# stevengiacalone/triceratops

Hardware: AMD Instinct MI355X
Metric: light-curve-point x sample evals/sec (higher is better)
Workload: dtype f64

## Files before the change

include/trx_debug.h:

```cpp
#ifndef TRX_DEBUG_H
#define TRX_DEBUG_H

#include "trx.h"

#ifdef __cplusplus
extern "C" {
#endif

int trx_set_rows_per_wave(int rows);
int trx_set_cell_packing_below(int n_time);
int trx_debug_batch_plan(long rows, int rows_per_wave, int taper, long* positions, int* rows_min);

int trx_set_supersample_tiers(int on);
int trx_set_stencil(int on);
int trx_set_skip_excluded(int on);
int trx_set_debug_node_counts(int on);
int trx_set_kepler_stepping(int on);

int trx_set_bounded_evaluation(int mode);
int trx_set_debug_bounded_lnl(int on);
int trx_set_debug_poison(int on);
int trx_set_debug_bug(int on);
int trx_set_probe_rows(int rows);
int trx_set_star_chain(int on);
int trx_set_row_order(int on);
int trx_debug_row_order(long* n_rows, long* segment_capacity, int* counts, int* lists, double* row_blocks);
int trx_set_whole_trips(int on);
int trx_debug_whole_trips(long* whole, long* walked, int reset);
int trx_debug_chain_counts(long* chains, long* calls_in_chains, long* posterior_calls_in_chains, int reset);

int trx_debug_select_from_halfchi2(const double* halfchi2, const double* lnprior, const double* cols,
                                   const double* cols_pad, long n, long N, long n_total, int ncol, int twin, int K,
                                   int moments, double lnsigma, double* out_record, double* out_post_x,
                                   double* out_table, void* stream);

int trx_debug_capture_buffers(long* live, long* idle);

#ifdef __cplusplus
}
#endif
#endif
```

triceratops_amd/_lib.py:

```python
import ctypes
import os
import threading

import numpy as np
import torch

_HERE = os.path.dirname(os.path.abspath(__file__))
LIB_PATH = os.environ.get("TRX_LIB") or os.path.join(_HERE, "libtrx.so")
TESTING_LIB_PATH = os.environ.get("TRX_TESTING_LIB") or os.path.join(_HERE, "libtrx_testing.so")

MODEL_TP, MODEL_EB, MODEL_EB_TWIN, MODEL_RAW = 0, 1, 2, 3
FLAG_COMPANION_IS_HOST, FLAG_SCALAR_K, FLAG_FP32_MODEL, FLAG_EVALUATE_EXCLUDED = 1, 2, 4, 8
FLAG_ALL_SUBEXPOSURES, FLAG_NO_STENCIL, FLAG_COUNT_EVALUATIONS, FLAG_FULL_EVALUATION = 16, 32, 64, 128
FLAG_WEIGHT_MOMENTS = 256
N_PARAM = {MODEL_TP: 10, MODEL_EB: 11, MODEL_EB_TWIN: 11, MODEL_RAW: 9}
ERR_NTOTAL = 4

ABI_SYMBOLS = (
    "trx_lnl_batch", "trx_lnl_batch_weighted", "trx_flux_grid", "trx_chi2_grid", "trx_chi2_grid_weighted",
    "trx_chi2_grid_offset", "trx_chi2_grid_baseline", "trx_workspace_bytes",
    "trx_log_mean_exp", "trx_lnz_scenario", "trx_lnz_from_halfchi2", "trx_lnz_moments_from_halfchi2",
    "trx_posterior_from_halfchi2", "trx_grid_quantiles",
    "trx_lnl_batch_host", "trx_flux_grid_host",
    "trx_log_mean_exp_host", "trx_skipped_rows", "trx_pruned_rows",
    "trx_draw_scenario", "trx_draw_args_size", "trx_scenario_evidence", "trx_scenario_enqueue", "trx_star_enqueue",
    "trx_scenario_args_size", "trx_release_scratch", "trx_version", "trx_last_error", "trx_device_count",
)
WARP_SYMBOLS = ("trxw_hist_from_halfchi2",)
NOISE_SYMBOLS = ("trxn_chi2_grid_ou",)
MIX_SYMBOLS = ("trxm_chi2_grid_ou_mix",)
SHIFT_SYMBOLS = ("trxt_softmin_rows",)
DEBUG_SYMBOLS = (
    "trx_set_rows_per_wave", "trx_set_cell_packing_below", "trx_debug_batch_plan", "trx_set_supersample_tiers",
    "trx_set_stencil", "trx_set_skip_excluded", "trx_set_debug_node_counts", "trx_set_kepler_stepping",
    "trx_set_bounded_evaluation", "trx_set_debug_bounded_lnl", "trx_set_debug_poison", "trx_set_debug_bug",
    "trx_set_probe_rows", "trx_set_star_chain", "trx_debug_capture_buffers", "trx_debug_chain_counts",
    "trx_set_row_order", "trx_debug_row_order", "trx_set_whole_trips", "trx_debug_whole_trips",
    "trx_debug_select_from_halfchi2",
)


class TrxError(RuntimeError):
    pass


EXTRA_FLAGS = 0
CELL_PACKING_BELOW = 320
STATS = {"rows": 0, "cells": 0, "launches": 0, "native_calls": 0}
_stats_lock = threading.Lock()


def count_launch(rows, n_time):
    with _stats_lock:
        STATS["rows"] += rows
        STATS["cells"] += rows * n_time
        STATS["launches"] += 1
TRACE = None
TRACE_SAMPLE_ROWS = 128


def reset_stats():
    for k in STATS:
        STATS[k] = 0


def set_precision(mode):
    global EXTRA_FLAGS
    if mode not in ("fp64", "fp32"):
        raise ValueError("precision must be 'fp64' or 'fp32'")
    EXTRA_FLAGS = (EXTRA_FLAGS & ~FLAG_FP32_MODEL) | (FLAG_FP32_MODEL if mode == "fp32" else 0)


def set_full_evaluation(on):
    global EXTRA_FLAGS
    EXTRA_FLAGS = (EXTRA_FLAGS | FLAG_FULL_EVALUATION) if on else (EXTRA_FLAGS & ~FLAG_FULL_EVALUATION)


_vp = ctypes.c_void_p
_lib = None
_production = None
_testing = None


def lib():
    global _lib, _production
    if _lib is not None:
        return _lib
    if os.environ.get("TRX_TESTING") == "1":
        return use_testing_library(True)
    if _production is None:
# ... 40 lines not shown
    L.trx_chi2_grid_weighted.restype = c_int
    L.trx_chi2_grid_weighted.argtypes = [_vp, _vp, _vp, c_int, c_long, _vp, c_double, c_int, _vp, _vp]
    L.trx_chi2_grid_offset.restype = c_int
    L.trx_chi2_grid_offset.argtypes = [_vp, _vp, _vp, c_int, c_long, _vp, c_double, c_int, _vp, c_double, c_double, _vp,
                                       _vp]
    L.trx_chi2_grid_baseline.restype = c_int
    L.trx_chi2_grid_baseline.argtypes = [_vp, _vp, _vp, c_int, c_long, _vp, c_double, c_int, _vp, _vp, c_int, _vp, _vp,
                                         _vp]
    L.trx_workspace_bytes.restype = c_size_t
    L.trx_workspace_bytes.argtypes = []
    L.trx_log_mean_exp.restype = c_int
    L.trx_log_mean_exp.argtypes = [_vp, c_long, c_long, _vp, _vp, c_size_t, _vp]
    L.trx_lnz_scenario.restype = c_int
    L.trx_lnz_scenario.argtypes = [c_int, c_int, _vp, _vp, c_int, c_double, _vp, c_long, c_double,
                                   c_int, _vp, c_long, c_double, _vp, _vp, _vp, c_size_t, _vp]
    L.trx_lnz_from_halfchi2.restype = c_int
    L.trx_lnz_from_halfchi2.argtypes = [_vp, _vp, c_long, c_long, c_double, _vp, _vp, c_size_t, _vp]
    L.trx_lnz_moments_from_halfchi2.restype = c_int
    L.trx_lnz_moments_from_halfchi2.argtypes = [_vp, _vp, c_long, c_long, c_double, _vp, _vp, c_size_t, _vp]
    L.trx_posterior_from_halfchi2.restype = c_int
    L.trx_posterior_from_halfchi2.argtypes = [_vp, _vp, c_long, c_double, c_int, ctypes.c_ulonglong, _vp, _vp, _vp,
                                              c_size_t, _vp]
    L.trxw_hist_from_halfchi2.restype = c_int
    L.trxw_hist_from_halfchi2.argtypes = [_vp, _vp, _vp, _vp, c_long, c_double, _vp, _vp, c_size_t, _vp]
    L.trxn_chi2_grid_ou.restype = c_int
    L.trxn_chi2_grid_ou.argtypes = [_vp, _vp, c_int, c_long, _vp, c_double, c_int, _vp, _vp, _vp, _vp, _vp]
    L.trxm_chi2_grid_ou_mix.restype = c_int
    L.trxm_chi2_grid_ou_mix.argtypes = [_vp, _vp, c_int, c_long, _vp, c_double, c_int, _vp, _vp, _vp, _vp, c_int, _vp, _vp,
                                        _vp]
    L.trxt_softmin_rows.restype = c_int
    L.trxt_softmin_rows.argtypes = [_vp, c_long, c_long, c_int, _vp, c_int, _vp, _vp]
    L.trx_grid_quantiles.restype = c_int
    L.trx_grid_quantiles.argtypes = [_vp, c_long, c_int, _vp, _vp, c_long, _vp, c_int, _vp, _vp]
    L.trx_lnl_batch_host.restype = c_int
    L.trx_lnl_batch_host.argtypes = [c_int, c_int, _vp, _vp, c_int, c_double, _vp, c_long,
                                     c_double, c_int, _vp]
    L.trx_flux_grid_host.restype = c_int
    L.trx_flux_grid_host.argtypes = [c_int, c_int, _vp, c_int, _vp, c_long, c_double, c_int, _vp, _vp]
    L.trx_log_mean_exp_host.restype = c_int
    L.trx_log_mean_exp_host.argtypes = [_vp, c_long, c_long, _vp]
    L.trx_skipped_rows.restype = c_int
    L.trx_skipped_rows.argtypes = [ctypes.POINTER(ctypes.c_ulonglong), c_int]
    L.trx_pruned_rows.restype = c_int
    L.trx_pruned_rows.argtypes = [ctypes.POINTER(ctypes.c_ulonglong), c_int]
    L.trx_version.restype = ctypes.c_char_p
    L.trx_last_error.restype = ctypes.c_char_p
    L.trx_device_count.restype = c_int
    L.trx_testing = bool(testing)
    if testing:
        for name in ("trx_set_rows_per_wave", "trx_set_kepler_stepping", "trx_set_skip_excluded",
                     "trx_set_bounded_evaluation", "trx_set_debug_bounded_lnl", "trx_set_debug_poison",
                     "trx_set_debug_bug", "trx_set_star_chain", "trx_set_probe_rows", "trx_set_stencil",
                     "trx_set_supersample_tiers", "trx_set_debug_node_counts", "trx_set_cell_packing_below",
                     "trx_set_row_order", "trx_set_whole_trips"):
            fn = getattr(L, name)
            fn.restype = c_int
            fn.argtypes = [c_int]
        L.trx_debug_capture_buffers.restype = c_int
        L.trx_debug_capture_buffers.argtypes = [ctypes.POINTER(c_long), ctypes.POINTER(c_long)]
        L.trx_debug_row_order.restype = c_int
        L.trx_debug_row_order.argtypes = [ctypes.POINTER(c_long), ctypes.POINTER(c_long), _vp, _vp, _vp]
        L.trx_debug_whole_trips.restype = c_int
        L.trx_debug_whole_trips.argtypes = [ctypes.POINTER(c_long), ctypes.POINTER(c_long), c_int]
        L.trx_debug_select_from_halfchi2.restype = c_int
        L.trx_debug_select_from_halfchi2.argtypes = [_vp, _vp, _vp, _vp, c_long, c_long, c_long, c_int, c_int, c_int, c_int,
                                                     c_double, _vp, _vp, _vp, _vp]
    return L


def check(rc):
    if rc:
        msg = lib().trx_last_error().decode()
        if rc == ERR_NTOTAL:
            raise ValueError(msg)
        raise TrxError("libtrx error %d: %s" % (rc, msg))


def version():
    return lib().trx_version().decode()


_gpu_seen = False


def require_gpu():
    global _gpu_seen
    if _gpu_seen:
        return
    if not torch.cuda.is_available() or lib().trx_device_count() < 1:
        raise TrxError("triceratops_amd needs an AMD GPU (gfx950); none is visible and there is no "
                       "CPU fallback")
    _gpu_seen = True
    from . import hw_queues
    if hw_queues()["in_effect"] is False:
        import warnings
        warnings.warn("triceratops_amd was imported after the HIP runtime had been initialised: GPU_MAX_HW_QUEUES=16 "
                      "did not take effect (the runtime keeps its default of 4 hardware queues; calc_probs on more "
                      "than two streams runs ~10 % slower).  Import triceratops_amd before the first GPU call or "
                      "export GPU_MAX_HW_QUEUES=16.", RuntimeWarning, stacklevel=3)


def compute_device():
    require_gpu()
    return torch.device("cuda", torch.cuda.current_device())


_upload_streams = {}
# ... 455 lines not shown
```

triceratops_amd/csrc/trx_cells.hpp:

```cpp
#pragma once
#include <hip/hip_runtime.h>
#include <math.h>

#include <cstddef>
#include <cstdint>

#include "../../include/trx.h"
#include "trx_device.hpp"
#include "trx_internal.hpp"

namespace {

using namespace trx;

constexpr int MODE_LNL = 0;
constexpr int MODE_GRID = 1;

struct RowsArgs {
    int model, flags;
    const double* time;
    const double* flux;
    int n_time;
    double sigma;
    const double* params;
    long n;
    double exptime;
    int S;
    double* out;
    double* out_sec;
    int B;
    long nbatch;
    int use_tiers, debug_nodes;
    int debug_bug;
    int need_sec;
    int mark_unwritten;
    int use_stencil;
    int skip_excl;
    int* memo;
    int tl_off;
    int wave_off, wave_doubles;
    int probe_rows;
    int wave_floor;
    int wave_floor3;
    double* rowc;
    int* scan_list;
    unsigned long long* scan_count;
    const long* n_dev;
    const int* src_idx;
    long src_stride;
    int twin_cols;
    int dense;
    int forced_B;
    int prune;
    int pstride;
    int pstride3;
    double prune_c0;
    const double* prune_lp;
    int part;
    int split;
    int* surv_list;
    unsigned long long* surv_count;
    int* probe_list;
    unsigned long long* probe_count;
    TierHead tiers;
    const double* tier_xw;
    double s2, rs2, dS, rS;
    const double* inv_var;
    double sec_limit;
    int accumulate;
    int whole_trips;
    int* order;
};

#ifndef TRX_CHAIN_MAX_BRANCHES
#define TRX_CHAIN_MAX_BRANCHES 24
#endif
struct BranchArgs {
    int model, flags, twin_cols, need_sec;
    const double* flux;
    double sigma, s2, rs2, prune_c0;
    const double* params;
    double* out;
    const long* n_dev;
    const int* src_idx;
    const double* prune_lp;
    double* scratch;
    unsigned long long* scan_count;
};
constexpr int kChainMaxBranches = TRX_CHAIN_MAX_BRANCHES;
struct BranchTab {
    BranchArgs b[kChainMaxBranches];
};
static_assert(sizeof(RowsArgs) + sizeof(BranchTab) + 16 <= 4096, "kernel argument buffer");

__device__ __forceinline__ double uniform(double v)
{
    const unsigned long long b = __double_as_longlong(v);
    const unsigned lo = __builtin_amdgcn_readfirstlane((unsigned)b);
    const unsigned hi = __builtin_amdgcn_readfirstlane((unsigned)(b >> 32));
    return __longlong_as_double(((unsigned long long)hi << 32) | lo);
}

__device__ __forceinline__ long uniform_long(long v)
{
    const unsigned lo = __builtin_amdgcn_readfirstlane((unsigned)(unsigned long long)v);
    const unsigned hi = __builtin_amdgcn_readfirstlane((unsigned)((unsigned long long)v >> 32));
    return (long)(((unsigned long long)hi << 32) | lo);
}

__device__ __forceinline__ bool mask_bit(unsigned long long m, int i)
{
    const unsigned w = (i & 32) ? (unsigned)(m >> 32) : (unsigned)m;
    return ((w >> (i & 31)) & 1u) != 0u;
}

__device__ __forceinline__ long row_pos(const RowsArgs& a, long row)
{
    if (a.dense) return a.twin_cols ? a.src_stride - 1 - row : row;
    return a.src_idx ? (long)a.src_idx[row] : row;
}

__device__ __forceinline__ int lanes_below(unsigned long long m)
{
    return __builtin_amdgcn_mbcnt_hi((unsigned)(m >> 32), __builtin_amdgcn_mbcnt_lo((unsigned)m, 0u));
}

#ifdef TRX_PHASE_TIMERS
__device__ unsigned long long g_phase_cycles[8];
#define TRX_TICK(var) const unsigned long long var = __builtin_readcyclecounter()
#define TRX_TOCK(slot, from) tm[slot] += __builtin_readcyclecounter() - (from)
#else
#define TRX_TICK(var)
#define TRX_TOCK(slot, from)
#endif

#ifdef TRX_TAIL_TIMERS
constexpr int kTailWaves = 1 << 17;
__device__ unsigned long long g_tail[4] = {~0ull, 0ull, 0ull, 0ull};
__device__ unsigned long long g_tail_finish[kTailWaves];
#endif

constexpr int kStatShards = 256, kStatPad = 16;
__device__ unsigned long long g_row_stats[2][kStatShards][kStatPad];
__device__ __forceinline__ void add_row_stat(int which, unsigned count)
{
    if (count) atomicAdd(&g_row_stats[which][(blockIdx.x + 41u * blockIdx.y) & (kStatShards - 1)][0], (unsigned long long)count);
}

#ifdef TRX_TESTING
__device__ unsigned long long g_trip_stats[2][kStatShards][kStatPad];
__device__ __forceinline__ void add_trip_stat(int which, unsigned count)
{
    if (count) atomicAdd(&g_trip_stats[which][(blockIdx.x + 41u * blockIdx.y) & (kStatShards - 1)][0], (unsigned long long)count);
}
__device__ __forceinline__ bool whole_trips_on(const RowsArgs& a) { return a.whole_trips != 0; }
#define TRX_TRIP_STAT(var) ++var
#else
__device__ __forceinline__ bool whole_trips_on(const RowsArgs&) { return true; }
#define TRX_TRIP_STAT(var)
#endif

__device__ __forceinline__ double k_rule(double k, bool scalar_rule)
{
    if (scalar_rule) { if (fabs(k - 1.0) < 1e-6) k *= 0.999; }
    else             { if ((k - 1.0) < 1e-6) k *= 0.999; }
    return k;
}

#ifndef TRX_BATCH_WAVES
#define TRX_BATCH_WAVES 4
#endif

constexpr int kBatchWaves = TRX_BATCH_WAVES;
__host__ __device__ constexpr int cells_waves(bool long_rows) { return long_rows ? 1 : kBatchWaves; }
#ifndef TRX_TIER_LDS
#define TRX_TIER_LDS(PRUNE, LONG) true
#endif
#ifndef TRX_ATAN_TAB
#define TRX_ATAN_TAB(PRUNE, LONG) (((PRUNE) && !(LONG)) ? 2 : 1)
#endif
#ifndef TRX_LONG_ROWS_IN_LDS
#define TRX_LONG_ROWS_IN_LDS 0
#endif
#ifndef TRX_CARRY_CELLS
#define TRX_CARRY_CELLS 1
#endif
#ifndef TRX_CELLS_WAVES_PER_EU
#define TRX_CELLS_WAVES_PER_EU 4
#endif
#ifndef TRX_LAZY_TIERS
#define TRX_LAZY_TIERS 1
#endif
#ifndef TRX_CELLS_PAIRS
#define TRX_CELLS_PAIRS 640
#endif
#ifndef TRX_CELLS_WINDOW
#define TRX_CELLS_WINDOW 2048
#endif
constexpr int kCellsMaxRows = 22;
#ifndef TRX_CELLS_WINDOW_BATCH
#define TRX_CELLS_WINDOW_BATCH 768
#endif
#ifndef TRX_BATCH_WAVES_PER_EU
#define TRX_BATCH_WAVES_PER_EU 5
#endif
constexpr int kCellsWindowLong = TRX_CELLS_WINDOW, kCellsWindowBatch = TRX_CELLS_WINDOW_BATCH;
static_assert(kCellsWindowLong % 64 == 0 && kCellsWindowLong <= 64 * 64, "window_trips: a lane per trip, windows that begin on a trip");
__host__ __device__ constexpr int cells_window(bool long_rows) { return long_rows ? kCellsWindowLong : kCellsWindowBatch; }
constexpr int kCellsPairs = TRX_CELLS_PAIRS;

__host__ __device__ inline int batch_rows(long n, int n_time, int forced, int floor = 3200)
{
    int B = (640 + n_time / 2) / (n_time > 0 ? n_time : 1);
    B = B < 1 ? 1 : (B > kCellsMaxRows ? kCellsMaxRows : B);
    if (forced > 0) return forced > kCellsMaxRows ? kCellsMaxRows : forced;
    if (n >= 0)
        while (B > 1 && n / B < floor) B = (B + 1) / 2;
    return B;
}

#ifndef TRX_TAPER_SLOTS
#define TRX_TAPER_SLOTS 320
#endif
struct BatchPlan {
    long R;
    long ra, rb;
    long pa, pb, P;
    int B, B2, B3;
};
__host__ __device__ inline BatchPlan batch_plan(long rows, int B, bool taper = true)
{
    BatchPlan p;
    p.B = B;
    p.B2 = (B + 1) / 2;
    p.B3 = B / 4 > 0 ? B / 4 : 1;
    const long nb = (rows + B - 1) / B;
    p.R = ((nb + 7) / 8) * B;
    long rb = 0, rc = 0;
#ifndef TRX_NO_TAPER
    if (B > 1 && taper) {
        constexpr long kSlotsPerXcd = TRX_TAPER_SLOTS;
        rc = kSlotsPerXcd * p.B3;
        if (rc > (3 * p.R) / 20) rc = (3 * p.R) / 20;
        rb = kSlotsPerXcd * p.B2;
        if (rb > (3 * p.R) / 10) rb = (3 * p.R) / 10;
        rc -= rc % B;
        rb -= rb % B;
// ... 878 lines not shown
                const int cell = c0 + lane;
                const bool valid = cell < win1;
                if (ST && !((trips >> ((c0 - win0) >> 6)) & 1ull)) {
                    if (MODE == MODE_GRID && valid) a.out[(size_t)base * n_time + cell] = a.debug_nodes ? 0.0 : hmout[0];
                    continue;
                }
                if (kWholeTrips && ((trips >> (32 + ((c0 - win0) >> 6))) & 1ull)) {
                    if (MODE == MODE_GRID && a.debug_nodes && valid) a.out[(size_t)base * n_time + cell] = 0.0;
                    if (valid) winlist[nw + lanes_below(~0ull)] = (unsigned short)(cell - win0);
                    nw += (win1 - c0 < 64) ? win1 - c0 : 64;
                    TRX_TRIP_STAT(n_whole);
                    continue;
                }
                TRX_TRIP_STAT(n_walked);
                int rr = 0, j = valid ? cell : 0;
                if (!LONG) {
                    rr = valid ? (int)(((float)cell + 0.5f) * inv_nt) : (nb - 1);
                    rr = rr < nb ? rr : nb - 1;
                    j = valid ? (cell - rr * n_time) : 0;
                }
                bool inw = false;
                TRX_CENSUS_ADD(kCenWindowTrip, 1);
                if (PRUNE && !LONG && !__any(valid && !mask_bit(skipmask, rr))) continue;
                if (valid) {
                    const RowC& c = (LONG && !TRX_LONG_ROWS_IN_LDS) ? cu : rows[rr];
                    const double phase = c.nmot * (tl[j] - c.t0);
                    const double dMc = reduce_2pi(phase);
                    const double slack = 1e-15 * fabs(phase);
                    const RowC& cw = rows[rr];
                    inw = in_window(cw.wlo - slack, cw.whi + slack, dMc) && !mask_bit(skipmask, rr);
                    if (MODE == MODE_GRID && (!inw || a.debug_nodes))
                        a.out[(size_t)base * n_time + cell] = a.debug_nodes ? 0.0 : hmout[rr];
                    if (LONG && MODE == MODE_LNL && !inw && phase_no == 0) {
                        const double d = fl[j] - 1.0;
                        lacc = fma(d * d, WT ? wl[j] : rs2, lacc);
                    }
                    if (PRUNE) {
                        if (!LONG && inw && phase_no == 0) {
                            const double d = fl[j] - 1.0;
                            __hip_atomic_fetch_add(&hrem[rr], (d * d) * rs2, __ATOMIC_RELAXED, __HIP_MEMORY_SCOPE_WORKGROUP);
                        }
                        if (nphase == 2) {
                            const bool probe = (j % pstride) == (pstride >> 1);
                            inw = inw && (probe == (phase_no == 0));
                        }
                    }
                }
                const unsigned long long mw = __ballot(inw);
                if (inw) winlist[nw + lanes_below(mw)] = (unsigned short)(cell - win0);
                nw += __popcll(mw);
            }
            wave_sync();
            TRX_TOCK(1, t_p1);
            int nheavy = 0;
            for (int sweep = 0; sweep < 2; ++sweep) {
            const int count = sweep ? nheavy : nw;
            const bool halo = ST && sweep == 0 && st_radius > 0.0;
            int carry_j = 0;
            unsigned long long carry_ok = 0;
            int ncarry = 0;
            for (int w0 = 0, step = 64; w0 < count || (kCarry && ncarry > 0); w0 += step) {
                TRX_TICK(t_plan);
                TRX_CENSUS_ADD(sweep ? kCenChunk1 : kCenChunk0, 1);
                bool owned = true;
                const bool carried = kCarry && lane < ncarry;
                if (kCarry) step = 64 - ncarry;
                const int csrc = (lane + 64 - ncarry) & 63;
                const unsigned cmeta = carried ? cs.meta[csrc] : 0u;
                bool valid = carried ? (cmeta & 0x20000u) != 0 : (w0 + lane - ncarry) < count;
                int rel = (int)*(carried ? &cs.rel[csrc] : &winlist[valid ? (w0 + lane - ncarry) : (count - 1)]);
                bool last_chunk = false;
                if (ST && halo) {
                    last_chunk = w0 + 64 >= count;
                    step = last_chunk ? 64 : 64 - kStM;
                    owned = lane < step;
                    if (w0 > 0 && lane < kStM) ss.fc[lane] = ss.fc[kStM + (64 - 2 * kStM) + lane];
                    wave_sync();
                }
                const int cell = win0 + rel;
                int rr = 0, j = cell;
                if (!LONG) {
                    rr = (int)(((float)cell + 0.5f) * inv_nt);
                    rr = rr < nb ? rr : nb - 1;
                    j = cell - rr * n_time;
                }
                const double t = tl[j];
                double fobs = 0.0;
                if (LONG && MODE == MODE_LNL) fobs = fl[j];
                double wobs = rs2;
                if (LONG && WT) wobs = wl[j];
                CellPlan pl;
                if (carried) {
                    pl.n = (int)(cmeta >> 18); pl.tier = (int)((cmeta >> 8) & 0xffu) - 1;
                    pl.sE = cs.sE[csrc]; pl.cE = cs.cE[csrc];
                    pl.anchored = (cmeta & 0x10000u) != 0;
                } else if (valid) {
                    const RowC& c = (LONG && !TRX_LONG_ROWS_IN_LDS) ? cu : rows[rr];
#ifndef TRX_PLAN_FULL_SOLVE
                    if (LONG && sweep == 1) pl = plan_all_subexposures<PRUNE>(c, t, a.S);
                    else
#endif
                    pl = plan_cell<false, PRUNE, TRX_TIER_LDS(PRUNE, LONG), kLazyTiers>(c, t, a.exptime, a.S, a.tiers, a.use_tiers != 0,
                                                                                        (ST && sweep == 0) ? st_radius : 0.0, thead);
                    if (STEP && !pl.anchored && pl.n > 0) {
                        kepler_full(c.nmot * (t - c.t0) + c.Mtr, c.e, pl.sE, pl.cE);
                        pl.anchored = true;
                    }
                }
                if (sweep == 0 && a.use_tiers) {
                    const bool heavy = valid && !pl.lazy && pl.tier < 0 && pl.n > 0;
                    const unsigned long long mh = __ballot(heavy && owned);
                    if (heavy && owned) winlist[nheavy + lanes_below(mh)] = (unsigned short)rel;
                    if (heavy) { pl.n = 0; valid = false; }
                    nheavy += __popcll(mh);
                }
                int tier = pl.tier;
                int nodes = (valid && owned) ? pl.n : 0;
                bool st = false, centre = false;
                if (ST && sweep == 0) {
                    const int jleft = __shfl(carry_j, 64 - 2 * kStM + lane, 64), jhere = __shfl(j, lane - kStM, 64);
                    const int jm = (lane < kStM) ? jleft : jhere;
                    const int jp = __shfl(j, lane + kStM, 64);
                    const unsigned long long mok = __ballot(valid);
                    const unsigned long long left = (carry_ok >> (64 - 2 * kStM)) & ((1ull << kStM) - 1ull);
                    const bool inner = (lane >= kStM || (halo && w0 > 0)) && lane + kStM < 64;
                    constexpr unsigned long long kAll = (1ull << (2 * kStM + 1)) - 1ull;
                    const unsigned long long field = (lane >= kStM) ? (mok >> (lane - kStM)) : (((mok << kStM) | left) >> lane);
                    st = inner && owned && valid && pl.n > 0 && pl.st_ok && jm == j - kStM && jp == j + kStM &&
                         (field & kAll) == kAll;
                    const unsigned long long mst = __ballot(st);
                    unsigned long long dil = mst;
#pragma unroll
                    for (int i = 1; i <= kStM; ++i) dil |= (mst << i) | (mst >> i);
                    centre = valid && ((dil >> lane) & 1ull);
                    const unsigned long long mnext = __ballot(valid && pl.n > 0 && pl.st_ok) >> (64 - kStM);
                    const int kk = lane - (64 - 2 * kStM);
                    if (halo && !last_chunk && valid && !centre && kk >= 0 && kk < kStM && (mnext & ((2ull << kk) - 1ull)) != 0) {
                        if (pl.n > 0) centre = true;
                        else ss.fc[kStM + lane] = 1.0;
                    }
                    if (st) nodes = 0;
                    carry_j = j;
                    carry_ok = mok;
                    if (kLazyTiers) {
                        const bool need = pl.lazy && nodes > 0;
                        if (__any(need)) {
                            if (need) {
                                const RowC& c = (LONG && !TRX_LONG_ROWS_IN_LDS) ? cu : rows[rr];
                                plan_tiers(c, a.exptime, pl, thead);
                                tier = pl.tier;
                                nodes = pl.n;
                            }
                        }
                    }
                }
                const bool direct = kLazyTiers && ST && sweep == 0 && !__any(nodes > 0);
                if (direct) {
                    if (centre) {
                        const RowC& c = (LONG && !TRX_LONG_ROWS_IN_LDS) ? cu : rows[rr];
                        const double ce = pl.cE - c.e;
                        const double X = fma(c.ax, ce, c.bx * pl.sE);
                        const double Y = fma(c.ay, ce, c.by * pl.sE);
                        const double yc = Y * c.cosi;
                        const double z2 = fma(X, X, yc * yc);
                        const double opp = 1.0 + c.k;
                        double f = 1.0;
                        if (Y >= 0.0 && z2 < opp * opp) {
                            const Limb L{c.cle, c.cld, c.ced};
                            f = disc_flux<FP32, TRX_ATAN_TAB(PRUNE, LONG)>(sqrt_fast(z2), c.k, L, atab);
                        } else if (z2 != z2) {
                            f = z2;
                        }
                        ss.fc[kStM + lane] = f;
                    }
                    wave_sync();
                }
                if (kCarry) wave_sync();
                if (!direct) {
                    cs.sE[lane] = pl.sE; cs.cE[lane] = pl.cE;
                    cs.t[lane] = t;
                    cs.facc[lane] = 0.0;
                    cs.meta[lane] = (unsigned)rr | ((unsigned)(tier + 1) << 8) | (pl.anchored ? 0x10000u : 0u) |
                                    (valid ? 0x20000u : 0u) | ((unsigned)pl.n << 18);
                    if (kCarry) cs.rel[lane] = (unsigned short)rel;
                }
                TRX_TOCK(2, t_plan);
                TRX_TICK(t_a);
                int ldone = 64;
                const int ncells = __popcll(__ballot(nodes > 0 || (ST && centre)));
                int per = ncells > 0 ? kCellsPairs / ncells - (ST ? 1 : 0) : kCellsPairs;
                per = per > 1000 ? 1000 : (per < 1 ? 1 : per);
                for (int s0 = 0; !direct && __any(s0 < nodes || (ST && s0 == 0 && centre)); s0 += per) {
                    int cnt = nodes - s0;
                    cnt = cnt < 0 ? 0 : (cnt > per ? per : cnt);
                    TRX_CENSUS_ADD(kCenPass, 1);
                    const int extra = (ST && s0 == 0 && centre) ? 1 : 0;
                    int total;
                    const int off = (sweep == 0 && a.use_tiers) ? lane_prefix<4>(cnt + extra, total)
                                                                : lane_prefix<10>(cnt + extra, total);
                    for (int si = 0; si < cnt; ++si) pdesc[off + si] = (unsigned short)(lane | (si << 6));
                    if (extra) pdesc[off + cnt] = (unsigned short)(lane | (kCentreNode << 6));
                    wave_sync();
                    if (kCarry && !(ST && halo) && s0 == 0 && w0 + step < count && total >= 64 && !__any(nodes > per)) {
                        const int whole = total & ~63;
                        const int l0 = __popcll(__ballot(off + cnt + extra <= whole));
                        if (l0 >= 1 && l0 < 64 && (64 - (total - whole)) > (64 - l0)) {
                            ldone = l0;
                            total = __builtin_amdgcn_readlane(off, l0);
                        }
                    }
                    for (int p0 = 0; p0 < total; p0 += 64) {
                        const int p = p0 + lane;
                        TRX_CENSUS_ADD(kCenPairTrip, 1);
                        TRX_CENSUS_ADD(kCenPairLanes, (unsigned long long)(total - p0 < 64 ? total - p0 : 64));
                        if (p < total) {
                            const int d = (int)pdesc[p];
                            const int h = d & 63;
                            const bool at_centre = ST && (d >> 6) == kCentreNode;
                            const int s = at_centre ? 0 : s0 + (d >> 6);
                            const unsigned meta = cs.meta[h];
                            const RowC& c = (LONG && !TRX_LONG_ROWS_IN_LDS) ? cu : rows[meta & 0xffu];
                            const int ht = (int)((meta >> 8) & 0xffu) - 1;
                            double sE = cs.sE[h], cE = cs.cE[h];
                            if (!at_centre) {
                                const double frac = (ht < 0) ? fma((double)(s + 1) - 0.5, a.rS, -0.5)
                                                             : tier_xw[2 * (ht * kTierMaxNodes + s)];
                                const double dM = c.nmot * (a.exptime * frac);
                                bool have = false;
                                if (STEP && (meta & 0x10000u)) have = kepler_step<PRUNE>(dM, c.e, sE, cE);
                                if (!have) {
                                    TRX_CENSUS_ADD(kCenKeplerFullPair, 1);
                                    kepler_full(c.nmot * ((cs.t[h] + a.exptime * frac) - c.t0) + c.Mtr, c.e, sE, cE);
                                }
                            }
                            const double ce = cE - c.e;
                            const double X = fma(c.ax, ce, c.bx * sE);
                            const double Y = fma(c.ay, ce, c.by * sE);
                            const double yc = Y * c.cosi;
                            const double z2 = fma(X, X, yc * yc);
                            const double opp = 1.0 + c.k;
                            double f = 1.0;
                            if (Y >= 0.0 && z2 < opp * opp) {
                                const Limb L{c.cle, c.cld, c.ced};
                                f = disc_flux<FP32, TRX_ATAN_TAB(PRUNE, LONG)>(sqrt_fast(z2), c.k, L, atab);
                            } else if (z2 != z2) {
                                f = z2;
                            }
                            if (at_centre) {
                                ss.fc[kStM + h] = f;
                            } else {
                                const double term = (ht < 0) ? f : tier_xw[2 * (ht * kTierMaxNodes + s) + 1] * (1.0 - f);
                                if (ht < 0 || term != 0.0)
                                    __hip_atomic_fetch_add(&cs.facc[h], term, __ATOMIC_RELAXED, __HIP_MEMORY_SCOPE_WORKGROUP);
                            }
                        }
                    }
// ... 327 lines not shown
```

triceratops_amd/csrc/trx_kernels.hip:

```cpp
#include <hip/hip_runtime.h>
#include <math.h>
#include <stdio.h>
#include <stdlib.h>
#include <string.h>

#include <atomic>
#include <cstddef>
#include <cstdint>
#include <map>
#include <mutex>
#include <utility>
#include <vector>

#include "../../include/trx.h"
#include "../../include/trx_noise.h"
#include "../../include/trx_mix.h"
#include "../../include/trx_shift.h"
#include "trx_device.hpp"
#include "trx_internal.hpp"
#include "trx_knobs.hpp"

namespace {

using namespace trx;
// ... 207 lines not shown
    const dim3 g(grid), block(LONG ? 64 : 64 * kBatchWaves);
    if constexpr (!PRUNE && !WT) {
        if (!step) {
            hipLaunchKernelGGL((cells_kernel<MODE, false, false, LONG, ST, false, false>), g, block, lds, st, a);
            return;
        }
    }
    if (fp32) hipLaunchKernelGGL((cells_kernel<MODE, true, true, LONG, ST, PRUNE, WT>), g, block, lds, st, a);
    else      hipLaunchKernelGGL((cells_kernel<MODE, true, false, LONG, ST, PRUNE, WT>), g, block, lds, st, a);
}

template <int MODE>
void launch_pruned(const RowsArgs& a, hipStream_t st, bool long_rows, bool fp32, unsigned grid, size_t lds)
{
    if constexpr (MODE == MODE_LNL) {
        if (long_rows) launch_cells_kernel<MODE_LNL, true, false, true, false>(true, fp32, grid, lds, st, a);
        else           launch_cells_kernel<MODE_LNL, false, false, true, false>(true, fp32, grid, lds, st, a);
    }
}

bool short_rows(int n_time) { return n_time > 0 && n_time < knob_cells_below(); }

struct CellsPlan {
    bool long_rows, prune, split, fp32, step;
    size_t lds;
    unsigned grid_main;
    unsigned grid_pilot;
    unsigned grid_rowc;
    unsigned grid_scan;
    unsigned grid_screen;
    bool passes;
    int probe_B;
    size_t probe_lds;
    int probe_wave_doubles;
};

#ifndef TRX_PROBE_FP32
#define TRX_PROBE_FP32 1
#endif
constexpr bool kProbeFp32 = TRX_PROBE_FP32 != 0;

template <int MODE>
int plan_cells(RowsArgs& a, bool long_rows, CellsPlan& P)
{
    a.forced_B = knob_rows_per_wave();
    a.B = long_rows ? 1 : batch_rows(a.n_dev ? -1 : a.n, a.n_time, a.forced_B);
    a.s2 = a.sigma * a.sigma;
    a.rs2 = 1.0 / a.s2;
    a.dS = (double)a.S;
    a.rS = 1.0 / a.dS;
    a.nbatch = 8 * batch_plan(a.n, a.B).P;
    a.debug_bug = knob_debug_bug();
    a.whole_trips = knob_whole_trips();
    a.mark_unwritten = (MODE == MODE_LNL && !a.inv_var) ? 1 : 0;
    bool tiers_ok = false;
    if (tier_device(a.S, a.tiers, &a.tier_xw, &tiers_ok)) return fail(TRX_ERR_HIP, "tier table upload failed%s", "", 0);
    a.use_tiers = tiers_ok && knob_tiers() && !(a.flags & TRX_FLAG_ALL_SUBEXPOSURES);
    const int prune_mode = (a.flags & TRX_FLAG_FULL_EVALUATION) ? 0 : (a.prune == 2 ? 2 : knob_bounded());
    const bool prune = MODE == MODE_LNL && a.prune && knob_kepler_stepping() &&
                       (prune_mode == 2 || (prune_mode == 1 && long_rows)) &&
                       (long_rows || (long)a.B * a.n_time <= (long)kCellsWindowBatch) &&
                       a.n_time >= kProbeMinPoints;
    a.prune = prune ? 1 : 0;
    static const int probe_cells = (int)env_long("TRX_PROBE_CELLS", kProbeCells);
    a.pstride = prune ? (a.n_time / probe_cells > 1 ? a.n_time / probe_cells : 2) : 1;
    static const int third_stride = (int)env_long("TRX_THIRD_STRIDE", kThirdStride);
    a.pstride3 = (prune && third_stride > 1 && a.n_time >= 4 * third_stride) ? third_stride : 0;
    a.use_stencil = (!prune && long_rows && a.use_tiers && a.exptime > 0.0 && a.S >= 8 && a.n_time >= 64 &&
                     knob_stencil() && !(a.flags & TRX_FLAG_NO_STENCIL)) ? 1 : 0;
    a.skip_excl = knob_skip_excluded() && !(a.flags & TRX_FLAG_EVALUATE_EXCLUDED);
    a.need_sec = (a.model == TRX_MODEL_EB && MODE == MODE_LNL) ||
                 ((a.model == TRX_MODEL_EB || a.model == TRX_MODEL_EB_TWIN) && a.out_sec != nullptr);
    if (a.inv_var && !(a.sec_limit < INFINITY)) a.need_sec = 0;
    static_assert((kCellsPairs + kCellsWindowLong) % 4 == 0 && (kCellsPairs + kCellsWindowBatch) % 4 == 0 &&
                  sizeof(CellState) % 8 == 0 && sizeof(StencilState) % 8 == 0, "8-byte alignment of the LDS arrays");
    const size_t tables = (size_t)(2 * kTiers * kTierMaxNodes + kAtanRanges * kAtanCols + kTierHeadDoubles) * sizeof(double);
    auto wave_bytes = [&](bool long_variant) -> size_t {
        return (size_t)a.B * (kRowDoubles + 4) * sizeof(double)
             + (kCellsPairs + cells_window(long_variant)) * sizeof(unsigned short) + sizeof(CellState)
             + (long_variant ? sizeof(StencilState) : 0);
    };
    a.tl_off = (int)(tables / sizeof(double));
    size_t shared = tables + (long_rows ? 0 : (size_t)(a.inv_var ? 3 : 2) * a.n_time * sizeof(double));
    size_t lds = shared + cells_waves(long_rows) * wave_bytes(long_rows);
    if (lds > 64 * 1024) {
        long_rows = true;
        a.B = 1;
        a.nbatch = a.n;
        shared = tables;
        lds = shared + wave_bytes(true);
    }
    a.wave_off = (int)(shared / sizeof(double));
    a.wave_doubles = (int)(wave_bytes(long_rows) / sizeof(double));
#ifdef TRX_NO_SPLIT
    const bool split = false;
#else
    const bool split = prune && !long_rows;
#endif
    a.split = split ? 1 : 0;
    P.probe_B = a.B;
    P.probe_lds = lds;
    P.probe_wave_doubles = a.wave_doubles;
    a.probe_rows = 0;
    a.wave_floor = a.wave_floor3 = 3200;
    if (split && knob_probe_rows() != 1) {
        const int forced = knob_probe_rows();
// ... 955 lines not shown
    g_knob_debug_bug = on ? 1 : 0;
    return TRX_OK;
}

int trx_set_probe_rows(int rows)
{
    if (rows < 0 || rows > kCellsMaxRows) return fail(TRX_ERR_ARG, "probe rows must be 0 (automatic) .. 22%s (got %ld)", "", (long)rows);
    g_knob_probe_rows = rows;
    return TRX_OK;
}

int trx_set_debug_bounded_lnl(int on)
{
    g_knob_bounded_lnl = on ? 1 : 0;
    return TRX_OK;
}

int trx_set_stencil(int on)
{
    g_knob_stencil = on ? 1 : 0;
    return TRX_OK;
}

int trx_set_kepler_stepping(int on)
{
    g_knob_kepler_stepping = on ? 1 : 0;
    return TRX_OK;
}

int trx_set_supersample_tiers(int on)
{
    g_knob_tiers = on ? 1 : 0;
    return TRX_OK;
}

int trx_set_debug_node_counts(int on)
{
    g_knob_debug_nodes = on ? 1 : 0;
    return TRX_OK;
}

int trx_set_row_order(int on)
{
    g_knob_row_order = on ? 1 : 0;
    return TRX_OK;
}

int trx_set_whole_trips(int on)
{
    g_knob_whole_trips = on ? 1 : 0;
    return TRX_OK;
}

int trx_debug_whole_trips(long* whole, long* walked, int reset)
{
    static unsigned long long host[2][kStatShards][kStatPad];
    static std::mutex mu;
    std::lock_guard<std::mutex> lock(mu);
    TRX_HIP(hipDeviceSynchronize());
    TRX_HIP(hipMemcpyFromSymbol(host, HIP_SYMBOL(g_trip_stats), sizeof(host), 0));
    long sum[2] = {0, 0};
    for (int w = 0; w < 2; ++w)
        for (int i = 0; i < kStatShards; ++i) sum[w] += (long)host[w][i][0];
    if (whole) *whole = sum[0];
    if (walked) *walked = sum[1];
    if (reset) {
        memset(host, 0, sizeof(host));
        TRX_HIP(hipMemcpyToSymbol(HIP_SYMBOL(g_trip_stats), host, sizeof(host), 0));
    }
    return TRX_OK;
}

int trx_debug_row_order(long* n_rows, long* segment_capacity, int* counts, int* lists, double* row_blocks)
{
    if (!t_last_order || !t_last_rowc) return fail(TRX_ERR_ARG, "trx_debug_row_order: no ordered launch yet%s", "", 0);
    const long n = t_last_order_rows, cap = order_cap(n);
    if (n_rows) *n_rows = n;
    if (segment_capacity) *segment_capacity = cap;
    if (!counts && !lists && !row_blocks) return TRX_OK;
    TRX_HIP(hipDeviceSynchronize());
    if (counts) {
        std::vector<int> raw((size_t)kOrderSegs * kOrderStride);
        TRX_HIP(hipMemcpy(raw.data(), t_last_order, raw.size() * sizeof(int), hipMemcpyDeviceToHost));
        for (int sgm = 0; sgm < kOrderSegs; ++sgm) counts[sgm] = raw[(size_t)sgm * kOrderStride];
    }
    if (lists)
        TRX_HIP(hipMemcpy(lists, t_last_order + kOrderSegs * kOrderStride, (size_t)kOrderSegs * cap * sizeof(int), hipMemcpyDeviceToHost));
    if (row_blocks)
        TRX_HIP(hipMemcpy(row_blocks, t_last_rowc, (size_t)n * kRowDoubles * sizeof(double), hipMemcpyDeviceToHost));
    return TRX_OK;
}

int trx_debug_capture_buffers(long* live, long* idle)
{
    long a = 0, b = 0;
    trx::capture_scratch_stats(&a, &b);
    if (live) *live = a;
    if (idle) *idle = b;
    return TRX_OK;
}

#endif

#ifdef TRX_CENSUS
int trx_debug_census(unsigned long long* out32, int reset)
{
// ... 66 lines not shown
```

triceratops_amd/csrc/trx_knobs.hpp:

```cpp
#pragma once
#include <stdlib.h>

#ifdef TRX_TESTING
#include <atomic>
#endif

namespace trx {

#ifdef TRX_TESTING
inline int knob_env_int(const char* name, int dflt)
{
    const char* e = name ? getenv(name) : nullptr;
    return (e && *e) ? atoi(e) : dflt;
}
inline long env_long(const char* name, long dflt)
{
    const char* e = getenv(name);
    return (e && *e) ? atol(e) : dflt;
}
inline double env_double(const char* name, double dflt)
{
    const char* e = getenv(name);
    return (e && *e) ? atof(e) : dflt;
}
#define TRX_KNOB(name, dflt, env)                                              \
    inline std::atomic<int> g_knob_##name{knob_env_int(env, dflt)};           \
    inline int knob_##name() { return g_knob_##name.load(std::memory_order_relaxed); }
#else
constexpr long env_long(const char*, long dflt) { return dflt; }
constexpr double env_double(const char*, double dflt) { return dflt; }
#define TRX_KNOB(name, dflt, env) \
    constexpr int knob_##name() { return dflt; }
#endif

TRX_KNOB(rows_per_wave, 0, nullptr)
TRX_KNOB(probe_rows, 0, "TRX_PROBE_ROWS")
TRX_KNOB(kepler_stepping, 1, nullptr)
TRX_KNOB(tiers, 1, nullptr)
TRX_KNOB(bounded, 2, "TRX_BOUNDED")
TRX_KNOB(bounded_lnl, 0, nullptr)
TRX_KNOB(skip_excluded, 1, nullptr)
TRX_KNOB(stencil, 1, nullptr)
TRX_KNOB(debug_nodes, 0, nullptr)
TRX_KNOB(cells_below, 320, nullptr)
TRX_KNOB(debug_bug, 0, nullptr)
TRX_KNOB(poison, 0, nullptr)
TRX_KNOB(star_chain, 1, "TRX_STAR_CHAIN")
TRX_KNOB(row_order, 1, nullptr)
TRX_KNOB(whole_trips, 1, nullptr)

#undef TRX_KNOB

}
```

Measured before the change: 50.10 billion.

## Fold heavy-row second sweep into one cell-packed sweep for long LNL rows

For long, non-pruned likelihood rows, heavy (untiered) points are no longer deferred to a second sweep. Instead all points are handled in a single sweep, and node work is packed into fixed-capacity pair batches by walking lanes (lane0) until the pair buffer fills. This removes the second pass over the window list and its extra wave syncs and bookkeeping, at the cost of a different packing loop, wider prefix sums, and possibly less balanced batches. A testing knob and debug setter are added to toggle the behaviour.

After: 51.51 billion (median of 6 runs). 1.03x the previous value.

```diff
diff --git a/include/trx_debug.h b/include/trx_debug.h
--- a/include/trx_debug.h
+++ b/include/trx_debug.h
@@ -26,6 +26,7 @@
 int trx_set_row_order(int on);
 int trx_debug_row_order(long* n_rows, long* segment_capacity, int* counts, int* lists, double* row_blocks);
 int trx_set_whole_trips(int on);
+int trx_set_one_sweep(int mode);
 int trx_debug_whole_trips(long* whole, long* walked, int reset);
 int trx_debug_chain_counts(long* chains, long* calls_in_chains, long* posterior_calls_in_chains, int reset);
 
diff --git a/profiles/one_sweep/measure.py b/profiles/one_sweep/measure.py
--- /dev/null
+++ b/profiles/one_sweep/measure.py
@@ -0,0 +1,116 @@
+import json
+import os
+import shutil
+import subprocess
+import sys
+import tempfile
+
+import numpy as np
+
+R = os.path.dirname(os.path.dirname(os.path.dirname(os.path.abspath(__file__))))
+PY = sys.executable
+
+
+def run(cmd, limit, lib, **kw):
+    env = dict(os.environ, TRX_LIB=lib)
+    p = subprocess.run(["timeout", "-k", "10", str(limit)] + cmd, cwd=R, env=env, stdout=subprocess.PIPE, text=True, **kw)
+    if p.returncode != 0:
+        print("FAILED (%d): %s" % (p.returncode, " ".join(cmd)))
+        print(p.stdout[-2000:])
+        sys.exit(1)
+    return p.stdout
+
+
+def last_json(text):
+    return json.loads(text.strip().splitlines()[-1])
+
+
+def census(parent_census):
+    for n_time, grid in ((2000, "uniform"), (2000, "irregular")):
+        c = last_json(run([PY, "profiles/r05/census_run.py", str(n_time), grid], 240, parent_census))
+        rows = c["rows"]
+        print("parent census, %d %s points, per row: first-sweep chunks %.3f, second-sweep chunks %.3f, passes %.3f, "
+              "pair trips %.3f, lanes per pair trip %.2f" % (n_time, grid, c["chunk0"] / rows, c["chunk1"] / rows,
+                                                             c["pass"] / rows, c["pair_trip"] / rows, c["pair_lanes"] / c["pair_trip"]))
+        sys.stdout.flush()
+
+
+def ab(parent, tree):
+    rec = {"parent": [], "tree": []}
+    for rep in (1, 2, 3):
+        for arm, lib in (("parent", parent), ("tree", tree)):
+            d = last_json(run([PY, "bench.py", "--gpus", "1", "--full", "--steps", "10", "--warmup", "3", "--no-cpu-baseline",
+                               "--no-e2e", "--pmc", "off"], 400, lib))
+            sh, b = d.get("shapes") or {}, d.get("batch") or {}
+            row = {"cfg1": d["roofline"]["mean_launch_ms"], "value": d["value"], "ms_per_step": d["ms_per_step"],
+                   "irregular": (sh.get("n2000_irregular") or {}).get("mean_launch_ms", float("nan")),
+                   "n100": (sh.get("n100") or {}).get("mean_launch_ms", float("nan")),
+                   "n200": (sh.get("n200") or {}).get("mean_launch_ms", float("nan")),
+                   "toi64": b.get("ms_per_step", float("nan")),
+                   "evals": d["roofline"].get("model_evaluations_per_cell"), "checksum": d["lnZ_checksum"]}
+            rec[arm].append(row)
+            print("%-6s rep %d  cfg1 %.4f ms  value %.4e/s  ms_per_step %.3f | irregular %.4f ms | n100 %.4f n200 %.4f | "
+                  "64-TOI step %.2f ms | evaluations per cell %s | lnZ_checksum %.15g"
+                  % (arm, rep, row["cfg1"], row["value"], row["ms_per_step"], row["irregular"], row["n100"], row["n200"],
+                     row["toi64"], row["evals"], row["checksum"]))
+            sys.stdout.flush()
+    for key in ("cfg1", "ms_per_step", "irregular", "n100", "n200", "toi64"):
+        p, t = (np.array([r[key] for r in rec[a]]) for a in ("parent", "tree"))
+        spread = max(p.max() - p.min(), t.max() - t.min())
+        print("%-11s parent %.4f (spread %.4f)  tree %.4f (spread %.4f)  tree - parent %+.4f = %+.2f %% = %.1f within-arm spreads"
+              % (key, p.mean(), p.max() - p.min(), t.mean(), t.max() - t.min(), t.mean() - p.mean(),
+                 100.0 * (t.mean() - p.mean()) / p.mean(), (p.mean() - t.mean()) / spread if spread > 0 else float("inf")))
+
+
+def counters(parent, tree):
+    out = tempfile.mkdtemp(prefix="one_sweep_pmc_")
+    try:
+        for arm, lib in (("parent", parent), ("tree", tree)):
+            d = os.path.join(out, "pmc_" + arm)
+            run(["rocprofv3", "--pmc", "SQ_INSTS_VALU", "SQ_ACTIVE_INST_VALU", "SQ_BUSY_CYCLES", "SQ_WAVE_CYCLES",
+                 "--output-format", "csv", "-d", d, "--", PY, "profiles/r07/cells2000_once.py"], 240, lib, stderr=subprocess.STDOUT)
+            text = run([PY, "profiles/pmc_summary.py", d], 120, lib, stderr=subprocess.STDOUT)
+            print("== counters, %s" % arm)
+            lines = text.splitlines()
+            for i, line in enumerate(lines):
+                if "cells_kernel" in line and "<0" in line.replace(" ", ""):
+                    print("\n".join(lines[i:i + 5]))
+            sys.stdout.flush()
+    finally:
+        shutil.rmtree(out, ignore_errors=True)
+
+
+def outputs(parent, tree):
+    out = tempfile.mkdtemp(prefix="one_sweep_dump_")
+    try:
+        ck = {}
+        for arm, lib in (("parent", parent), ("tree", tree)):
+            d = last_json(run([PY, "bench.py", "--gpus", "1", "--steps", "2", "--warmup", "1", "--no-cpu-baseline",
+                               "--dump-outputs", os.path.join(out, arm)], 300, lib))
+            ck[arm] = d["lnZ_checksum"]
+        print("lnZ_checksum parent %.17g tree %.17g equal: %s" % (ck["parent"], ck["tree"], ck["parent"] == ck["tree"]))
+        for name in ("halfchi2", "lnZ"):
+            a, b = (np.load(os.path.join(out, arm, name + ".npy")) for arm in ("parent", "tree"))
+            assert a.shape == b.shape
+            same = a.view(np.uint64) == b.view(np.uint64)
+            fin = np.isfinite(a) & np.isfinite(b) & (a != 0)
+            rel = np.abs(a[fin] - b[fin]) / np.abs(a[fin])
+            print("%s.npy %s: %d of %d values bit-identical, largest relative change %.3g, NaN / inf in the same places: %s"
+                  % (name, a.shape, same.sum(), a.size, rel.max() if rel.size else 0.0,
+                     np.array_equal(np.isnan(a), np.isnan(b)) and np.array_equal(np.isinf(a), np.isinf(b))))
+    finally:
+        shutil.rmtree(out, ignore_errors=True)
+
+
+if __name__ == "__main__":
+    stage, parent, tree = sys.argv[1], os.path.abspath(sys.argv[2]), os.path.abspath(sys.argv[3])
+    if stage == "census":
+        census(os.path.abspath(sys.argv[4]))
+    elif stage == "ab":
+        ab(parent, tree)
+    elif stage == "counters":
+        counters(parent, tree)
+    elif stage == "outputs":
+        outputs(parent, tree)
+    else:
+        sys.exit("unknown stage " + stage)
diff --git a/triceratops_amd/_lib.py b/triceratops_amd/_lib.py
--- a/triceratops_amd/_lib.py
+++ b/triceratops_amd/_lib.py
@@ -35,7 +35,7 @@
     "trx_set_stencil", "trx_set_skip_excluded", "trx_set_debug_node_counts", "trx_set_kepler_stepping",
     "trx_set_bounded_evaluation", "trx_set_debug_bounded_lnl", "trx_set_debug_poison", "trx_set_debug_bug",
     "trx_set_probe_rows", "trx_set_star_chain", "trx_debug_capture_buffers", "trx_debug_chain_counts",
-    "trx_set_row_order", "trx_debug_row_order", "trx_set_whole_trips", "trx_debug_whole_trips",
+    "trx_set_row_order", "trx_debug_row_order", "trx_set_whole_trips", "trx_debug_whole_trips", "trx_set_one_sweep",
     "trx_debug_select_from_halfchi2",
 )
 
@@ -182,7 +182,7 @@
                      "trx_set_bounded_evaluation", "trx_set_debug_bounded_lnl", "trx_set_debug_poison",
                      "trx_set_debug_bug", "trx_set_star_chain", "trx_set_probe_rows", "trx_set_stencil",
                      "trx_set_supersample_tiers", "trx_set_debug_node_counts", "trx_set_cell_packing_below",
-                     "trx_set_row_order", "trx_set_whole_trips"):
+                     "trx_set_row_order", "trx_set_whole_trips", "trx_set_one_sweep"):
             fn = getattr(L, name)
             fn.restype = c_int
             fn.argtypes = [c_int]
diff --git a/triceratops_amd/csrc/trx_cells.hpp b/triceratops_amd/csrc/trx_cells.hpp
--- a/triceratops_amd/csrc/trx_cells.hpp
+++ b/triceratops_amd/csrc/trx_cells.hpp
@@ -69,6 +69,7 @@
     double sec_limit;
     int accumulate;
     int whole_trips;
+    int one_sweep;
     int* order;
 };
 
@@ -154,9 +155,11 @@
     if (count) atomicAdd(&g_trip_stats[which][(blockIdx.x + 41u * blockIdx.y) & (kStatShards - 1)][0], (unsigned long long)count);
 }
 __device__ __forceinline__ bool whole_trips_on(const RowsArgs& a) { return a.whole_trips != 0; }
+__device__ __forceinline__ bool one_sweep_on(const RowsArgs& a, bool lnl) { return a.one_sweep >= (lnl ? 1 : 2); }
 #define TRX_TRIP_STAT(var) ++var
 #else
 __device__ __forceinline__ bool whole_trips_on(const RowsArgs&) { return true; }
+__device__ __forceinline__ bool one_sweep_on(const RowsArgs&, bool lnl) { return lnl; }
 #define TRX_TRIP_STAT(var)
 #endif
 
@@ -193,6 +196,12 @@
 #endif
 #ifndef TRX_CELLS_PAIRS
 #define TRX_CELLS_PAIRS 640
+#endif
+#ifndef TRX_ONE_SWEEP
+#define TRX_ONE_SWEEP 1
+#endif
+#ifndef TRX_ONE_SWEEP_BATCH
+#define TRX_ONE_SWEEP_BATCH 0
 #endif
 #ifndef TRX_CELLS_WINDOW
 #define TRX_CELLS_WINDOW 2048
@@ -1177,8 +1186,10 @@
             }
             wave_sync();
             TRX_TOCK(1, t_p1);
+            constexpr bool kOneSweep = TRX_ONE_SWEEP && (LONG || TRX_ONE_SWEEP_BATCH) && !PRUNE;
+            const bool one = kOneSweep && one_sweep_on(a, MODE == MODE_LNL);
             int nheavy = 0;
-            for (int sweep = 0; sweep < 2; ++sweep) {
+            for (int sweep = 0; sweep < (one ? 1 : 2); ++sweep) {
             const int count = sweep ? nheavy : nw;
             const bool halo = ST && sweep == 0 && st_radius > 0.0;
             int carry_j = 0;
@@ -1232,12 +1243,17 @@
                         pl.anchored = true;
                     }
                 }
+                bool planned = valid;
                 if (sweep == 0 && a.use_tiers) {
                     const bool heavy = valid && !pl.lazy && pl.tier < 0 && pl.n > 0;
-                    const unsigned long long mh = __ballot(heavy && owned);
-                    if (heavy && owned) winlist[nheavy + lanes_below(mh)] = (unsigned short)rel;
-                    if (heavy) { pl.n = 0; valid = false; }
-                    nheavy += __popcll(mh);
+                    if (one) {
+                        planned = valid && !heavy;
+                    } else {
+                        const unsigned long long mh = __ballot(heavy && owned);
+                        if (heavy && owned) winlist[nheavy + lanes_below(mh)] = (unsigned short)rel;
+                        if (heavy) { pl.n = 0; valid = false; planned = false; }
+                        nheavy += __popcll(mh);
+                    }
                 }
                 int tier = pl.tier;
                 int nodes = (valid && owned) ? pl.n : 0;
@@ -1246,21 +1262,21 @@
                     const int jleft = __shfl(carry_j, 64 - 2 * kStM + lane, 64), jhere = __shfl(j, lane - kStM, 64);
                     const int jm = (lane < kStM) ? jleft : jhere;
                     const int jp = __shfl(j, lane + kStM, 64);
-                    const unsigned long long mok = __ballot(valid);
+                    const unsigned long long mok = __ballot(planned);
                     const unsigned long long left = (carry_ok >> (64 - 2 * kStM)) & ((1ull << kStM) - 1ull);
                     const bool inner = (lane >= kStM || (halo && w0 > 0)) && lane + kStM < 64;
                     constexpr unsigned long long kAll = (1ull << (2 * kStM + 1)) - 1ull;
                     const unsigned long long field = (lane >= kStM) ? (mok >> (lane - kStM)) : (((mok << kStM) | left) >> lane);
-                    st = inner && owned && valid && pl.n > 0 && pl.st_ok && jm == j - kStM && jp == j + kStM &&
+                    st = inner && owned && planned && pl.n > 0 && pl.st_ok && jm == j - kStM && jp == j + kStM &&
                          (field & kAll) == kAll;
                     const unsigned long long mst = __ballot(st);
                     unsigned long long dil = mst;
 #pragma unroll
                     for (int i = 1; i <= kStM; ++i) dil |= (mst << i) | (mst >> i);
-                    centre = valid && ((dil >> lane) & 1ull);
-                    const unsigned long long mnext = __ballot(valid && pl.n > 0 && pl.st_ok) >> (64 - kStM);
+                    centre = planned && ((dil >> lane) & 1ull);
+                    const unsigned long long mnext = __ballot(planned && pl.n > 0 && pl.st_ok) >> (64 - kStM);
                     const int kk = lane - (64 - 2 * kStM);
-                    if (halo && !last_chunk && valid && !centre && kk >= 0 && kk < kStM && (mnext & ((2ull << kk) - 1ull)) != 0) {
+                    if (halo && !last_chunk && planned && !centre && kk >= 0 && kk < kStM && (mnext & ((2ull << kk) - 1ull)) != 0) {
                         if (pl.n > 0) centre = true;
                         else ss.fc[kStM + lane] = 1.0;
                     }
@@ -1313,20 +1329,36 @@
                 TRX_TICK(t_a);
                 int ldone = 64;
                 const int ncells = __popcll(__ballot(nodes > 0 || (ST && centre)));
+                const bool by_cells = one && a.S < kCellsPairs;
                 int per = ncells > 0 ? kCellsPairs / ncells - (ST ? 1 : 0) : kCellsPairs;
                 per = per > 1000 ? 1000 : (per < 1 ? 1 : per);
-                for (int s0 = 0; !direct && __any(s0 < nodes || (ST && s0 == 0 && centre)); s0 += per) {
+                if (by_cells) per = kCellsPairs;
+                int lane0 = ncells > 0 ? 0 : 64;
+                for (int s0 = 0; !direct && (by_cells ? lane0 < 64 : __any(s0 < nodes || (ST && s0 == 0 && centre)));
+                     s0 += by_cells ? 0 : per) {
                     int cnt = nodes - s0;
                     cnt = cnt < 0 ? 0 : (cnt > per ? per : cnt);
                     TRX_CENSUS_ADD(kCenPass, 1);
-                    const int extra = (ST && s0 == 0 && centre) ? 1 : 0;
+                    int extra = (ST && s0 == 0 && centre) ? 1 : 0;
+                    if (by_cells && lane < lane0) { cnt = 0; extra = 0; }
                     int total;
-                    const int off = (sweep == 0 && a.use_tiers) ? lane_prefix<4>(cnt + extra, total)
-                                                                : lane_prefix<10>(cnt + extra, total);
+                    int off;
+                    if (one) off = (a.S + 1 < 32) ? lane_prefix<5>(cnt + extra, total) : lane_prefix<10>(cnt + extra, total);
+                    else off = (sweep == 0 && a.use_tiers) ? lane_prefix<4>(cnt + extra, total) : lane_prefix<10>(cnt + extra, total);
+                    if (by_cells) {
+                        const unsigned long long mover = __ballot(off + cnt + extra > kCellsPairs);
+                        lane0 = 64;
+                        if (mover) {
+                            lane0 = __ffsll((long long)mover) - 1;
+                            total = __builtin_amdgcn_readlane(off, lane0);
+                            if (lane >= lane0) { cnt = 0; extra = 0; }
+                        }
+                    }
                     for (int si = 0; si < cnt; ++si) pdesc[off + si] = (unsigned short)(lane | (si << 6));
                     if (extra) pdesc[off + cnt] = (unsigned short)(lane | (kCentreNode << 6));
                     wave_sync();
-                    if (kCarry && !(ST && halo) && s0 == 0 && w0 + step < count && total >= 64 && !__any(nodes > per)) {
+                    if (kCarry && !(ST && halo) && s0 == 0 && w0 + step < count && total >= 64 && !__any(nodes > per) &&
+                        (!by_cells || lane0 == 64)) {
                         const int whole = total & ~63;
                         const int l0 = __popcll(__ballot(off + cnt + extra <= whole));
                         if (l0 >= 1 && l0 < 64 && (64 - (total - whole)) > (64 - l0)) {
diff --git a/triceratops_amd/csrc/trx_kernels.hip b/triceratops_amd/csrc/trx_kernels.hip
--- a/triceratops_amd/csrc/trx_kernels.hip
+++ b/triceratops_amd/csrc/trx_kernels.hip
@@ -283,6 +283,7 @@
     a.nbatch = 8 * batch_plan(a.n, a.B).P;
     a.debug_bug = knob_debug_bug();
     a.whole_trips = knob_whole_trips();
+    a.one_sweep = knob_one_sweep();
     a.mark_unwritten = (MODE == MODE_LNL && !a.inv_var) ? 1 : 0;
     bool tiers_ok = false;
     if (tier_device(a.S, a.tiers, &a.tier_xw, &tiers_ok)) return fail(TRX_ERR_HIP, "tier table upload failed%s", "", 0);
@@ -1344,6 +1345,13 @@
     return TRX_OK;
 }
 
+int trx_set_one_sweep(int mode)
+{
+    if (mode < 0 || mode > 2) return fail(TRX_ERR_ARG, "trx_set_one_sweep: mode must be 0, 1 or 2%s (got %ld)", "", (long)mode);
+    g_knob_one_sweep = mode;
+    return TRX_OK;
+}
+
 int trx_debug_whole_trips(long* whole, long* walked, int reset)
 {
     static unsigned long long host[2][kStatShards][kStatPad];
diff --git a/triceratops_amd/csrc/trx_knobs.hpp b/triceratops_amd/csrc/trx_knobs.hpp
--- a/triceratops_amd/csrc/trx_knobs.hpp
+++ b/triceratops_amd/csrc/trx_knobs.hpp
@@ -48,6 +48,7 @@
 TRX_KNOB(star_chain, 1, "TRX_STAR_CHAIN")
 TRX_KNOB(row_order, 1, nullptr)
 TRX_KNOB(whole_trips, 1, nullptr)
+TRX_KNOB(one_sweep, 1, nullptr)
 
 #undef TRX_KNOB
 
```
